# edamametechnologies/flodbadd

Hardware: AMD Instinct MI355X
Metric: Mpackets/s device-resident header parse + 5-tuple classify, 64B & IMIX frames (higher is better)
Workload: dtype u8; 1 GPU; C2: 1,048,576 x 64-B IPv4/TCP frames per GPU, device-resident (BASELINE configs[1]); rotated_batches=32, batches_per_launch_max=32, filter=GlobalOnly, parallelism=packet-index shards x1

## Files before the change

### flodbadd_amd/csrc/fb_capi.hip

```cpp
#include <stdarg.h>
#include <stdio.h>
#include <stdlib.h>
#include <string.h>

#include <algorithm>
#include <chrono>
#include <cmath>
#include <memory>
#include <mutex>
#include <new>
#include <thread>
#include <vector>

#include "fb_host.h"
#include "fb_internal.h"
#include "service_ports_default.inc"

using namespace fbk;

namespace fbk {

static thread_local char g_err[512] = "";

int set_err(int code, const char* fmt, ...) {
// ... 486 lines not shown
        return nullptr;
    }
    hipDeviceProp_t prop;
    if (hipGetDeviceProperties(&prop, device) != hipSuccess || strncmp(prop.gcnArchName, "gfx950", 6) != 0) {
        set_err(FB_ERR_NODEV, "device %d is not gfx950 (%s)", device, prop.gcnArchName);
        return nullptr;
    }
    DeviceGuard g(device);
    fb_ctx* c = new (std::nothrow) fb_ctx();
    if (!c) { set_err(FB_ERR_NOMEM, "fb_ctx"); return nullptr; }
    c->device = device;
    {
        int sb = 0;
        if (occupancy_parse_seg(&sb) != hipSuccess || sb < 1) sb = 1;
        c->seg_grid = std::min<uint32_t>((uint32_t)(sb * prop.multiProcessorCount), 1023u);
#ifndef FB_ASYNC_BPC
#define FB_ASYNC_BPC 1
#endif
        c->seg_grid_async = std::min<uint32_t>((uint32_t)(FB_ASYNC_BPC * prop.multiProcessorCount), c->seg_grid);
        int db = 0;
        if (occupancy_parse_dense(&db) != hipSuccess || db < 1) db = 1;
        c->dense_grid = std::min<uint32_t>((uint32_t)(db * prop.multiProcessorCount), 1023u);
    }
    c->h_cfg.reset(new (std::nothrow) DevConfig());
    bool ok = c->h_cfg != nullptr;
    if (ok) {
        memset(c->h_cfg.get(), 0, sizeof(DevConfig));
        memcpy(c->h_cfg->service_bitmap, cfg->service_bitmap ? cfg->service_bitmap : kDefaultServiceBitmap,
               FB_SERVICE_BITMAP_BYTES);
        c->h_cfg->filter = cfg->filter;
        set_lan(c->h_cfg.get(), cfg->lan_v6, cfg->n_lan_v6);
        c->h_cfg->n_own = cfg->n_own_ips;
        for (uint32_t i = 0; i < cfg->n_own_ips; ++i) c->h_cfg->own[i] = cfg->own_ips[i];
    }
    ok = ok && c->d_cfg.alloc(1) == hipSuccess;
    ok = ok && c->d_error.alloc(4) == hipSuccess && hipMemset(c->d_error, 0, 16) == hipSuccess;
    ok = ok && c->d_tick.alloc(kTickWords) == hipSuccess && hipMemset(c->d_tick, 0, kTickWords * 8ull) == hipSuccess;
    ok = ok && c->d_n.alloc(2) == hipSuccess;
    if (ok && cfg->flow_capacity > kFlowMaxCapacity) {
        set_err(FB_ERR_INVAL, "flow_capacity %llu > %llu slots", (unsigned long long)cfg->flow_capacity,
                (unsigned long long)kFlowMaxCapacity);
        ok = false;
    }
    if (ok && cfg->flow_capacity) {
        uint64_t cap = kFlowSlots;
        while (cap < cfg->flow_capacity) cap <<= 1;
        ok = table_alloc(c->tb, cap, nullptr) == nullptr &&
             hipMemset(c->tb.slots, 0, cap * sizeof(FlowSlot)) == hipSuccess &&
             c->mbox.alloc(1, hipHostMallocMapped) == hipSuccess;
        if (ok) memset(c->mbox.get(), 0, sizeof(FlowMailbox));
        c->grow = (cfg->flags & FB_CFG_FIXED_TABLE) == 0u;
        c->timed = (cfg->flags & FB_CFG_TIMED) != 0u;
        if (ok && c->timed)
            ok = plane_ensure(c, kPlaneTime, nullptr) == FB_OK;
        ok = ok && ensure_flow_scratch(c, cfg->max_batch_packets, nullptr) == FB_OK;
    }
    ok = ok && upload_cfg(c, nullptr) == FB_OK;
    if (!ok) {
        if (g_err[0] == 0) set_err(FB_ERR_NOMEM, "device allocation failed");
        fb_destroy(c);
        return nullptr;
    }
    return c;
}

int fb_destroy(fb_ctx* c) {
    if (!c) return set_err(FB_ERR_INVAL, "ctx is NULL");
    DeviceGuard g(c->device);
    (void)hipDeviceSynchronize();
    dnstrack_free(c->dns);
    histstore_free(c->hs);
    delete c;
    return FB_OK;
}

int fb_set_filter(fb_ctx* c, uint32_t filter) {
    if (!c || filter > FB_FILTER_ALL) return set_err(FB_ERR_INVAL, "bad ctx or filter");
    if (c->h_cfg->filter != filter) { c->h_cfg->filter = filter; c->cfg_dirty = true; }
    return FB_OK;
}

int fb_set_service_bitmap(fb_ctx* c, const uint8_t* bm) {
    if (!c || !bm) return set_err(FB_ERR_INVAL, "bad ctx or bitmap");
    memcpy(c->h_cfg->service_bitmap, bm, FB_SERVICE_BITMAP_BYTES);
    c->cfg_dirty = true;
    return FB_OK;
}

int fb_set_lan_v6(fb_ctx* c, const fb_lan_v6* nets, uint32_t n) {
    if (!c || n > FB_MAX_LAN_V6 || (n && !nets)) return set_err(FB_ERR_INVAL, "bad lan_v6 table");
    set_lan(c->h_cfg.get(), nets, n);
    c->cfg_dirty = true;
    return FB_OK;
}

int fb_set_stage_event(fb_ctx* c, void* event) {
    if (!c) return set_err(FB_ERR_INVAL, "ctx is NULL");
    c->stage_event = (hipEvent_t)event;
    return FB_OK;
}

int fb_set_frame_times(fb_ctx* c, const uint64_t* d_ts) {
    if (!c) return set_err(FB_ERR_INVAL, "ctx is NULL");
    if (!c->timed) return set_err(FB_ERR_INVAL, "the context was created without FB_CFG_TIMED");
    c->next_ts = reinterpret_cast<const unsigned long long*>(d_ts);
    return FB_OK;
}

static int timed_ready(fb_ctx* c) {
    if (c->timed && !c->next_ts)
        return set_err(FB_ERR_INVAL, "a timed context needs fb_set_frame_times before each update call");
    return FB_OK;
}

int fb_debug_set(fb_ctx* c, uint32_t knob, uint64_t value) {
    if (!c) return set_err(FB_ERR_INVAL, "ctx is NULL");
    switch (knob) {
        case FB_DEBUG_DENSE_STEAL_POLLS:
            c->steal_polls = (uint32_t)std::min<uint64_t>(value, 0xFFFFFFFFull);
            return FB_OK;
        case FB_DEBUG_DENSE_OFFSET_SKEW:
            if (value > 0xFFFFFFFFull) return set_err(FB_ERR_INVAL, "skew %llu >= 2^32", (unsigned long long)value);
            c->dn_skew = value;
            if (value) fprintf(stderr, "flodbadd_gpu: FB_DEBUG_DENSE_OFFSET_SKEW %llu active on this context (fault injection)\n",
                               (unsigned long long)value);
            return FB_OK;
        case FB_DEBUG_VIEW_DIRECT:
            c->view_direct = value != 0;
            return FB_OK;
        case FB_DEBUG_ZEEK_DIRECT:
            c->zeek_direct = value != 0;
            return FB_OK;
        default:
            return set_err(FB_ERR_INVAL, "unknown debug knob %u", knob);
    }
}

int fb_set_session_records(fb_ctx* c, int emit) {
    if (!c) return set_err(FB_ERR_INVAL, "ctx is NULL");
    c->emit_records = emit != 0;
    return FB_OK;
}

int fb_set_own_ips(fb_ctx* c, const fb_ip* ips, uint32_t n) {
    if (!c || n > FB_MAX_OWN_IPS || (n && !ips)) return set_err(FB_ERR_INVAL, "bad own-ip table");
    c->h_cfg->n_own = n;
    for (uint32_t i = 0; i < n; ++i) c->h_cfg->own[i] = ips[i];
    c->cfg_dirty = true;
    return FB_OK;
}

#ifdef FB_SEG_TRACE
static unsigned long long* g_strace = nullptr;
extern "C" __attribute__((visibility("default"))) int fb_seg_trace_last(unsigned long long* out) {
    if (!g_strace || hipDeviceSynchronize() != hipSuccess) return -1;
    return hipMemcpy(out, g_strace, 8u * 4u * 2048u, hipMemcpyDeviceToHost) == hipSuccess ? 0 : -1;
}
#endif
static int launch_seg(fb_ctx* c, const SegBatches& sb, uint32_t n_max, const fb_parsed_pkt* parsed, hipStream_t s,
                      bool want_parts = false, SegPass pass = SegPass::kSegments, fb_pkt_out* dense_out = nullptr,
                      fb_dns_out* dense_dns = nullptr) {
    int rc = reset_launch_scratch(c, s);
    if (!rc && want_parts && !c->part_target) rc = join_updates(c, s);
    if (!rc) rc = upload_cfg(c, s);
    if (!rc) rc = ensure_flow_scratch(c, n_max, s);
    if (rc) return rc;
    c->last_n = n_max;
    ParseParams p;
    memset(&p, 0, sizeof(p));
    p.pre = c->sc.cpre;
    p.dense_out = dense_out;
    p.dense_dns = dense_dns;
    p.parsed = parsed;
    p.n = parsed ? sb.b[0].n : 0u;
    p.rec_part = (want_parts && sb.count == 1u && c->tb.slots) ? (c->part_target ? c->part_target : c->rs.rec_part.get())
                                                              : nullptr;
    p.rec_ent = p.rec_part ? (c->ent_target ? c->ent_target : c->rs.rec_ent.get()) : nullptr;
    p.no_records = p.rec_part && !c->emit_records ? 1u : 0u;
    p.part_shift = c->tb.shift;
    c->part_recs = p.rec_part ? sb.b[0].out : nullptr;
    c->part_buf = p.rec_part;
    c->ent_buf = p.rec_ent;
    p.cfg = c->d_cfg;
    p.tick = c->d_tick;
    if (pass != SegPass::kDenseOut) {
        rc = guard_next_error_word(c, s);
        if (rc) return rc;
    }
    const uint32_t launch = pass == SegPass::kDenseOut ? c->epoch : ++c->epoch;
    p.error = c->d_error + (launch & 3u);
    p.error_next = c->d_error + ((launch + 1u) & 3u);
    const uint32_t waves = parse_seg_block_threads() / 64u;
    const uint32_t grid = std::max<uint32_t>(1u, std::min<uint32_t>(c->seg_grid, (sb.total_segs + waves - 1) / waves));
#ifdef FB_SEG_TRACE
    if (!g_strace && hipMalloc(&g_strace, 8u * 4u * 2048u) != hipSuccess) return set_err(FB_ERR_NOMEM, "trace");
    HIP_TRY(hipMemsetAsync(g_strace, 0, 8u * 4u * 2048u, s));
    p.dtrace = g_strace;
#endif
    HIP_TRY(launch_parse_seg(p, sb, grid, s, pass));
    return FB_OK;
}

static SegBatches one_batch(const uint8_t* frames, uint64_t frames_bytes, const uint32_t* offsets, uint32_t n,
                            fb_pkt_out* out, uint32_t* seg, uint8_t* cls, fb_batch_stats* stats) {
    SegBatches sb;
    memset(&sb, 0, sizeof(sb));
    sb.count = 1;
    SegBatch& B = sb.b[0];
    B.frames = frames;
    B.offsets = offsets;
    B.out = out;
    B.seg = seg;
    B.cls = cls;
    B.stats = stats;
    B.n = n;
    B.frames_bytes = (uint32_t)frames_bytes;
    sb.total_segs = (n + FB_SEG_FRAMES - 1) / FB_SEG_FRAMES;
    return sb;
}

int fb_parse_classify_seg_batches_dev(fb_ctx* c, const fb_seg_batch* batches, uint32_t count, void* stream) {
    if (!c || !batches || count == 0 || count > FB_MAX_SEG_BATCHES)
        return set_err(FB_ERR_INVAL, "ctx, batches and 1 <= count <= FB_MAX_SEG_BATCHES are required");
    SegBatches sb;
    memset(&sb, 0, sizeof(sb));
    uint64_t segs = 0;
    uint32_t n_max = 0;
    for (uint32_t k = 0; k < count; ++k) {
        const fb_seg_batch& x = batches[k];
        if (!x.d_stats) return set_err(FB_ERR_INVAL, "batch %u: d_stats is required", k);
        if (x.n > FB_MAX_BATCH_PACKETS) return set_err(FB_ERR_INVAL, "batch %u: n > FB_MAX_BATCH_PACKETS", k);
        if (x.frames_bytes > 0xFFFFFFFFull) return set_err(FB_ERR_INVAL, "batch %u: frames_bytes must be < 4 GiB", k);
        if (!x.d_offsets || (x.n && (!x.d_out || !x.d_seg)))
            return set_err(FB_ERR_INVAL, "batch %u: d_offsets, d_out and d_seg are required", k);
        if (x.n && x.frames_bytes && !x.d_frames) return set_err(FB_ERR_INVAL, "batch %u: d_frames is NULL", k);
        SegBatch& B = sb.b[k];
        B.frames = x.d_frames;
        B.offsets = x.d_offsets;
        B.out = x.d_out;
        B.seg = x.d_seg;
        B.cls = x.d_class;
        B.stats = x.d_stats;
        B.n = x.n;
        B.frames_bytes = (uint32_t)x.frames_bytes;
        B.seg_start = (uint32_t)segs;
        segs += (x.n + FB_SEG_FRAMES - 1) / FB_SEG_FRAMES;
        n_max = std::max(n_max, x.n);
    }
    if (segs > 0xFFFFFFFFull / FB_SEG_FRAMES) return set_err(FB_ERR_INVAL, "too many frames in one launch");
    sb.count = count;
    sb.total_segs = (uint32_t)segs;
    DeviceGuard g(c->device);
    return launch_seg(c, sb, n_max, nullptr, (hipStream_t)stream);
}

#ifdef FB_DN_TRACE
static unsigned long long* g_dtrace = nullptr;
extern "C" __attribute__((visibility("default"))) int fb_dense_trace_last(unsigned long long* out) {
    if (!g_dtrace || hipDeviceSynchronize() != hipSuccess) return -1;
    return hipMemcpy(out, g_dtrace, 8u * 4u * (8192u + 1024u), hipMemcpyDeviceToHost) == hipSuccess ? 0 : -1;
}
#endif
#ifdef FB_QUEUE_TRACE
static unsigned long long g_qtrace[kQTraceAll];
#endif
struct fb_seg_queue {
    int device = 0;
    uint32_t depth = 0;
    uint32_t slots = 0;
    PinnedBuf<QueueHost> h;
    DevBuf<QueueDev> d_ring;
    DevBuf<DevConfig> d_cfg;
    DevBuf<unsigned long long> d_tick;
    DevBuf<uint32_t> d_blk;
    DevBuf<uint32_t> d_head;
    DevBuf<uint32_t> d_err;
    DevBuf<unsigned long long> d_trace;
    DevStream stream;
    uint64_t submitted = 0;
    uint64_t limit = FB_QUEUE_MAX_SUBMISSIONS;
    bool launched = false;
    hipError_t gone = hipSuccess;
    uint32_t grid = 0;
    uint64_t idle_ns = 0;
    std::chrono::steady_clock::time_point created;
    bool not_resident = false;
    bool counted = false;
};
static std::mutex g_queue_mu;
static uint32_t g_queue_live[64];

static void queue_free(fb_seg_queue* q) {
    if (q->counted) {
        std::lock_guard<std::mutex> lk(g_queue_mu);
        --g_queue_live[q->device];
    }
    delete q;
}

static uint64_t hload(const unsigned long long* p) { return __atomic_load_n(p, __ATOMIC_ACQUIRE); }

static int queue_kernel_gone(fb_seg_queue* q, uint64_t spin, uint64_t every) {
    if (hload(&q->h->status) & kQueueExpired) return FB_OK;
    if (spin % every != every - 1u) return 1;
    const hipError_t e = hipStreamQuery(q->stream);
    if (e == hipErrorNotReady) {
        if (hload(&q->h->pad[3]) != q->grid &&
            (uint64_t)std::chrono::duration_cast<std::chrono::nanoseconds>(std::chrono::steady_clock::now() -
                                                                          q->created).count() > q->idle_ns) {
            q->not_resident = true;
            return FB_OK;
        }
        return 1;
    }
    q->gone = e;
    return FB_OK;
}

static int queue_gone_error(fb_seg_queue* q) {
    const QueueHost* h = q->h;
    if (q->not_resident)
        return set_err(FB_ERR_INTERNAL,
                       "the queue kernel's blocks are not all running (%llu of %u started within idle_ms): the "
                       "device's CUs are held by other work; destroy the queue",
                       (unsigned long long)hload(&h->pad[3]), q->grid);
    return set_err(FB_ERR_INTERNAL,
                   "the queue kernel has stopped (status %llu, stream: %s; a block left after %llu ticks idle "
                   "waiting for batch %llu (block %llu), tail %llu): destroy the queue",
                   (unsigned long long)hload(&h->status), hipGetErrorString(q->gone), (unsigned long long)hload(&h->pad[0]),
                   (unsigned long long)(hload(&h->pad[1]) & 0xFFFFFFFFu), (unsigned long long)(hload(&h->pad[1]) >> 32),
                   (unsigned long long)hload(&h->pad[2]));
}

fb_seg_queue* fb_seg_queue_create(fb_ctx* c, uint32_t depth, uint32_t idle_ms) {
    return fb_seg_queue_create_ex(c, depth, idle_ms, 0u);
}

fb_seg_queue* fb_seg_queue_create_ex(fb_ctx* c, uint32_t depth, uint32_t idle_ms, uint32_t flags) {
    if (flags & ~FB_QUEUE_SHARED) {
        set_err(FB_ERR_INVAL, "unknown queue flags 0x%x", flags);
        return nullptr;
    }
    if (!c) {
        set_err(FB_ERR_INVAL, "ctx is NULL");
        return nullptr;
    }
    if (depth == 0u) depth = 8u;
    if (depth > kQueueMax) {
        set_err(FB_ERR_INVAL, "depth %u > FB_QUEUE_MAX_DEPTH", depth);
// ... 1740 lines not shown
```

### flodbadd_amd/csrc/fb_parse.hip

```cpp
#include "fb_internal.h"

namespace fbk {

typedef uint32_t u32x4 __attribute__((ext_vector_type(4)));
typedef uint32_t u32x2 __attribute__((ext_vector_type(2)));

#ifndef FB_LD_AUX
#define FB_LD_AUX 0
#endif
#ifndef FB_ST_AUX
#define FB_ST_AUX 2
#endif

__device__ __forceinline__ u32x4 ld16(__amdgpu_buffer_rsrc_t r, uint32_t off) {
    return __builtin_amdgcn_raw_buffer_load_b128(r, off, 0, FB_LD_AUX);
}

__device__ __forceinline__ uint32_t be16_lo(uint32_t w) { return ((w & 0xffu) << 8) | ((w >> 8) & 0xffu); }
__device__ __forceinline__ uint32_t be16_hi(uint32_t w) { return ((w >> 8) & 0xff00u) | (w >> 24); }
__device__ __forceinline__ uint32_t bswap(uint32_t w) { return __builtin_bswap32(w); }

__device__ __forceinline__ uint32_t svc(const uint32_t* bm, uint32_t p) { return (bm[p >> 5] >> (p & 31)) & 1u; }

__device__ __forceinline__ uint32_t hist_char(uint32_t fl, uint32_t plen, bool orig) {
    uint32_t c;
    if ((fl & 0x02u) && !(fl & 0x10u)) c = 'S';
    else if ((fl & 0x02u) && (fl & 0x10u)) c = 'H';
    else if (fl & 0x01u) c = 'F';
    else if (fl & 0x04u) c = 'R';
    else if (plen > 0u) c = '>';
    else if (fl & 0x10u) c = 'A';
    else return '-';
    if (c == '>') return orig ? '>' : '<';
    return orig ? c : c + 32u;
}

#ifndef FB_HDR_ALIGNED
#define FB_HDR_ALIGNED 1
#endif
struct Hdr {
#if FB_HDR_ALIGNED
    u32x4 A, B, C;
    uint32_t E;
    uint32_t D0, D1;
#else
    u32x4 A, B, C;
    uint32_t Dz;
#endif
};

__device__ __forceinline__ void hdr_view(const Hdr& h, uint32_t o, u32x4& A, u32x4& B, u32x4& C, uint32_t& Dz) {
#if FB_HDR_ALIGNED
    const uint32_t s = (o + 10u) & 3u;
    auto al = [s](uint32_t hi, uint32_t lo) { return __builtin_amdgcn_alignbyte(hi, lo, s); };
    A = u32x4{al(h.A.y, h.A.x), al(h.A.z, h.A.y), al(h.A.w, h.A.z), al(h.B.x, h.A.w)};
    B = u32x4{al(h.B.y, h.B.x), al(h.B.z, h.B.y), al(h.B.w, h.B.z), al(h.C.x, h.B.w)};
    C = u32x4{al(h.C.y, h.C.x), al(h.C.z, h.C.y), al(h.C.w, h.C.z), al(h.E, h.C.w)};
    Dz = al(h.D1, h.D0);
#else
    (void)o;
    A = h.A;
    B = h.B;
    C = h.C;
    Dz = h.Dz;
#endif
}

struct Pkt {
    uint32_t cls;
    uint32_t w[14];
    bool tcp, v4, bad;
};

__device__ __forceinline__ void classify_session(const DevConfig* cfg, const DevConfig* gcfg, uint32_t proto,
                                                 uint32_t fam, const uint32_t (&src)[4], const uint32_t (&dst)[4],
                                                 uint32_t sport, uint32_t dport, uint32_t hasf, uint32_t flags,
                                                 uint32_t plen, uint32_t iplen, uint32_t idx, Pkt& k) {
    const uint32_t* bm = cfg->service_bitmap;
    k.tcp = proto == 6u;
    k.v4 = fam == 2u;
    const uint32_t S = svc(bm, sport), Dsv = svc(bm, dport);
    bool swap;
    if (S && !Dsv) {
        swap = true;
    } else if (S && Dsv) {
        const bool tf = hasf && proto == 6u && (flags & 0x02u);
        if (tf && !(flags & 0x10u)) swap = false;
        else if (tf && (flags & 0x10u)) swap = true;
        else swap = sport < dport;
    } else {
        swap = false;
    }
    const bool orig = !swap || (src[0] == dst[0] && src[1] == dst[1] && src[2] == dst[2] &&
                                src[3] == dst[3] && sport == dport);
    uint32_t ks[4], kd[4];
#pragma unroll
    for (int j = 0; j < 4; ++j) {
        ks[j] = swap ? dst[j] : src[j];
        kd[j] = swap ? src[j] : dst[j];
    }
    const uint32_t kport_s = swap ? dport : sport, kport_d = swap ? sport : dport;
    const bool lan_s = fam == 2u ? lan_v4(ks[0]) : lan_v6(cfg, gcfg, ks);
    const bool lan_d = fam == 2u ? lan_v4(kd[0]) : lan_v6(cfg, gcfg, kd);
    uint32_t meta = hasf;
    meta |= swap ? FB_META_SWAP : 0u;
    meta |= orig ? FB_META_ORIGINATOR : 0u;
    meta |= lan_s ? FB_META_LOCAL_SRC : 0u;
    meta |= lan_d ? FB_META_LOCAL_DST : 0u;
    meta |= own_ip(cfg, gcfg, fam, ks) ? FB_META_SELF_SRC : 0u;
    meta |= own_ip(cfg, gcfg, fam, kd) ? FB_META_SELF_DST : 0u;
    meta |= (swap ? S : Dsv) ? FB_META_DST_SERVICE : 0u;
    const uint32_t hc = hasf ? hist_char(flags, plen, orig) : 0u;
#pragma unroll
    for (int j = 0; j < 4; ++j) {
        k.w[j] = ks[j];
        k.w[4 + j] = kd[j];
    }
    k.w[8] = kport_s | (kport_d << 16);
    k.w[9] = proto | (fam << 8);
    k.w[10] = plen;
    k.w[11] = iplen;
    k.w[12] = flags | (meta << 8) | (hc << 16);
    k.w[13] = idx;
    const bool local = lan_s && lan_d;
    const uint32_t f = cfg->filter;
    const bool drop = (f == FB_FILTER_LOCAL_ONLY && !local) || (f == FB_FILTER_GLOBAL_ONLY && local);
    k.cls = drop ? FB_CLASS_FILTERED : FB_CLASS_SESSION;
}

__device__ __forceinline__ void process_frame(__amdgpu_buffer_rsrc_t r, const DevConfig* cfg,
                                              const DevConfig* gcfg, const Hdr& h, uint32_t o0, uint32_t o1,
                                              uint32_t fbytes, uint32_t idx, Pkt& k) {
    k.cls = FB_CLASS_DROP;
    k.tcp = false;
    k.v4 = false;
    const bool okoff = o1 >= o0 && o1 <= fbytes;
    k.bad = !okoff;
    const uint32_t L = okoff ? o1 - o0 : 0u;
    u32x4 A, B, C;
    uint32_t Dz;
    hdr_view(h, o0, A, B, C, Dz);
    if (L < 14u) return;
    const uint32_t et = be16_hi(A.x);
    const uint32_t n = L - 14u;
    uint32_t src[4] = {0u, 0u, 0u, 0u}, dst[4] = {0u, 0u, 0u, 0u};
    uint32_t l4off, l4len, proto, d0, d3, iplen, fam;
    if (et == 0x0800u) {
        if (n < 20u) return;
        const uint32_t ihl4 = (A.y & 0xfu) * 4u;
        const uint32_t tot = be16_hi(A.y);
        proto = (A.w >> 8) & 0xffu;
        const uint32_t start = ihl4 > 20u ? ihl4 : 20u;
        const uint32_t plen = tot > ihl4 ? tot - ihl4 : 0u;
        l4len = n > start ? min(start + plen, n) - start : 0u;
        l4off = 14u + start;
        src[0] = bswap(B.x);
        dst[0] = bswap(B.y);
        iplen = tot;
        fam = 2u;
        if (start == 20u) {
            d0 = B.z;
            d3 = C.y;
        } else {
            const u32x4 E = ld16(r, o0 + l4off);
            d0 = E.x;
            d3 = E.w;
        }
    } else if (et == 0x86DDu) {
        if (n < 40u) return;
        const uint32_t plen6 = be16_lo(A.z);
        proto = (A.z >> 16) & 0xffu;
        src[0] = bswap(A.w); src[1] = bswap(B.x); src[2] = bswap(B.y); src[3] = bswap(B.z);
        dst[0] = bswap(B.w); dst[1] = bswap(C.x); dst[2] = bswap(C.y); dst[3] = bswap(C.z);
        l4off = 54u;
        l4len = n > 40u ? min(40u + plen6, n) - 40u : 0u;
        iplen = plen6 + 40u;
        fam = 10u;
        d0 = C.w;
        d3 = Dz;
    } else {
        return;
    }
    uint32_t sport, dport, flags = 0u, hasf = 0u, plen;
    if (proto == 6u) {
        if (l4len < 20u) return;
        sport = be16_lo(d0);
        dport = be16_hi(d0);
        const uint32_t doff = (d3 & 0xffu) >> 4;
        flags = (d3 >> 8) & 0xffu;
        hasf = 1u;
        const uint32_t hs = doff > 5u ? doff * 4u : 20u;
        plen = l4len <= hs ? 0u : l4len - hs;
        if (sport == 53u || dport == 53u) {
            if (plen < 2u) return;
            k.cls = FB_CLASS_DNS;
            k.w[0] = idx;
            k.w[1] = o0 + l4off + hs + 2u;
            k.w[2] = plen - 2u;
            k.w[3] = 6u | (fam << 8);
            return;
        }
    } else if (proto == 17u) {
        if (l4len < 8u) return;
        sport = be16_lo(d0);
        dport = be16_hi(d0);
        plen = l4len - 8u;
        if (sport == 53u || dport == 53u) {
            k.cls = FB_CLASS_DNS;
            k.w[0] = idx;
            k.w[1] = o0 + l4off + 8u;
            k.w[2] = plen;
            k.w[3] = 17u | (fam << 8);
            return;
        }
    } else {
        return;
    }

    classify_session(cfg, gcfg, proto, fam, src, dst, sport, dport, hasf, flags, plen, iplen, idx, k);
}

constexpr uint32_t kFlagsProduct = 0u;
constexpr uint32_t kPartOut = 8u;
constexpr uint32_t kCountOnly = 16u;
constexpr uint32_t kDense = 32u;


__device__ __forceinline__ void load_headers1(__amdgpu_buffer_rsrc_t rs, uint32_t o, Hdr& h) {
#if FB_HDR_ALIGNED
    const uint32_t a = (o + 10u) & ~3u;
    h.A = ld16(rs, a);
    h.B = ld16(rs, a + 16u);
    h.C = ld16(rs, a + 32u);
    h.E = __builtin_amdgcn_raw_buffer_load_b32(rs, a + 48u, 0, FB_LD_AUX);
    const u32x2 d = __builtin_amdgcn_raw_buffer_load_b64(rs, a + 56u, 0, FB_LD_AUX);
    h.D0 = d.x;
    h.D1 = d.y;
#else
    h.A = ld16(rs, o + 10u);
    h.B = ld16(rs, o + 26u);
    h.C = ld16(rs, o + 42u);
    h.Dz = __builtin_amdgcn_raw_buffer_load_b32(rs, o + 66u, 0, FB_LD_AUX);
#endif
}

__device__ __forceinline__ void lds_barrier() { asm volatile("s_waitcnt lgkmcnt(0)\n\ts_barrier" ::: "memory"); }

#ifndef FB_SEG_WAVES
#define FB_SEG_WAVES 8
#endif
#ifndef FB_SEG_BPC
#define FB_SEG_BPC 3
#endif
#ifndef FB_SEG_DEPTH
#define FB_SEG_DEPTH 1
#endif
constexpr int kSegWaves = FB_SEG_WAVES;
constexpr int kSegDepth = FB_SEG_DEPTH;
constexpr int kSegThreads = 64 * kSegWaves;
constexpr uint32_t kSegBytes = 64u * 56u;

#ifdef FB_SEG_TRACE
constexpr uint32_t kSegTrBlocks = 2048u;
__device__ __forceinline__ unsigned long long seg_now() {
    unsigned long long t;
    asm volatile("s_memrealtime %0\n\ts_waitcnt lgkmcnt(0)" : "=s"(t)::"memory");
    return t;
}
#define SEGTR(stmt) do { stmt; } while (0)
#else
#define SEGTR(stmt) do { } while (0)
#endif
template <bool PARSED, uint32_t FLAGS = kFlagsProduct, bool MULTI = false>
__global__ __launch_bounds__(kSegThreads, kSegWaves * FB_SEG_BPC / 4) void k_parse_seg(const ParseParams P,
                                                                                      const SegBatches SB) {
    const uint32_t tid = threadIdx.x, lane = tid & 63u;
    const uint32_t wave = __builtin_amdgcn_readfirstlane(tid >> 6);
    const uint32_t G = gridDim.x, b = blockIdx.x;
    const uint32_t nseg = SB.total_segs;
    const uint32_t nb = MULTI ? SB.count : 1u;
    constexpr uint32_t kAcc = kMaxSegBatches * 10u;
    __shared__ uint4 s_cfg4[sizeof(DevConfig) / 16];
    constexpr uint32_t kStageU64 = (FLAGS & kPartOut) ? 64u * 8u : 64u * 7u;
    __shared__ __attribute__((aligned(16))) unsigned long long s_stage[kSegWaves][kStageU64];
    __shared__ uint32_t s_acc[kAcc + 1];
    const DevConfig* cfg = reinterpret_cast<const DevConfig*>(s_cfg4);
    const unsigned long long lmask = (1ull << lane) - 1ull;
    unsigned long long* stage = s_stage[wave];
    uint32_t a_s = 0u, a_d = 0u, a_f = 0u, a_t = 0u, a_4 = 0u, a_b = 0u, a_n = 0u;
    uint32_t a_k = 0u;
    if (tid <= kAcc) s_acc[tid] = 0u;
    SEGTR(if (tid == 0u && b < kSegTrBlocks) P.dtrace[4u * b] = seg_now());

    uint32_t k_q = 0u, k_h = 0u, k_s = 0u;
    auto batch_of = [&](uint32_t& k, uint32_t g) {
        if constexpr (MULTI)
            while (k + 1u < nb && g >= SB.b[k + 1u].seg_start) ++k;
        return k;
    };
    auto frames_rsrc = [&](uint32_t k) {
        return __builtin_amdgcn_make_buffer_rsrc((void*)SB.b[k].frames, (short)0, (int)SB.b[k].frames_bytes, 0x00020000);
    };

    typedef uint32_t u32x2 __attribute__((ext_vector_type(2)));
    constexpr uint32_t kOob = 0x80000000u;
    const uint32_t stride = G * kSegWaves;
    const __amdgpu_buffer_rsrc_t r_drop = __builtin_amdgcn_make_buffer_rsrc(SB.b[0].seg, (short)0, 0, 0x00020000);
    auto vmov = [](uint32_t x) {
        uint32_t y;
        asm volatile("v_mov_b32 %0, %1" : "=v"(y) : "v"(x));
        return y;
    };
    constexpr int D = kSegDepth;
    static_assert(D == 1, "one segment of header loads in flight (dynamic hand-out)");
    __shared__ uint32_t s_next;
    auto seg_of = [&](uint32_t L) { return b * kSegWaves + L % kSegWaves + (L / kSegWaves) * stride; };
    auto grab = [&]() {
        uint32_t v = 0u;
        if (lane == 0u) v = __hip_atomic_fetch_add(&s_next, 1u, __ATOMIC_RELAXED, __HIP_MEMORY_SCOPE_WORKGROUP);
        return __builtin_amdgcn_readfirstlane(v);
    };
    struct Set {
        Hdr h;
        uint2 c, q;
        unsigned long long p;
    };
    Set SS[D];
    uint4 pin[4];
    auto load_q = [&](uint32_t g, uint2& q) {
        const uint32_t k = batch_of(k_q, g);
        const uint32_t i = (g - SB.b[k].seg_start) * 64u + lane, n = SB.b[k].n;
        const uint32_t* off = SB.b[k].offsets;
        q = make_uint2(off[min(i, n)], off[min(i + 1u, n)]);
    };
    auto load_pre = [&](uint32_t g) {
        return P.pre[min(g, nseg - 1u)];
    };
    unsigned long long ppre = 0ull;
    auto fetch = [&](Set& X, uint32_t g_h, uint32_t next_q) {
        if constexpr ((FLAGS & kDense) != 0u) X.p = load_pre(g_h);
        load_headers1(frames_rsrc(batch_of(k_h, g_h)), X.q.x, X.h);
        X.c = make_uint2(vmov(X.q.x), vmov(X.q.y));
        load_q(next_q, X.q);
    };
    constexpr int kStores = (FLAGS & kCountOnly) ? 2 : (FLAGS & kDense) ? 6 : ((FLAGS & kPartOut) ? 13 : 8);
    auto dropped_stores = [&]() {
#pragma unroll
        for (int j = 0; j < kStores; ++j) __builtin_amdgcn_raw_buffer_store_b32(0u, r_drop, kOob + 64u * j, 0, 0);
    };
    auto load_parsed = [&](uint32_t sg) {
        if constexpr ((FLAGS & kDense) != 0u) ppre = load_pre(sg);
        const uint32_t sc = min(sg, (P.n - 1u) >> 6);
        const uint32_t left = P.n - sc * 64u;
        const __amdgpu_buffer_rsrc_t rp = __builtin_amdgcn_make_buffer_rsrc(
            (void*)(P.parsed + (size_t)sc * 64u), (short)0, (int)(min(left, 64u) * 56u), 0x00020000);
        const uint32_t o = min(lane, left - 1u) * 56u;
        const u32x4 x0 = __builtin_amdgcn_raw_buffer_load_b128(rp, o, 0, 0);
        const u32x4 x1 = __builtin_amdgcn_raw_buffer_load_b128(rp, o + 16u, 0, 0);
        const u32x4 x2 = __builtin_amdgcn_raw_buffer_load_b128(rp, o + 32u, 0, 0);
        const u32x2 x3 = __builtin_amdgcn_raw_buffer_load_b64(rp, o + 48u, 0, 0);
        pin[0] = make_uint4(x0.x, x0.y, x0.z, x0.w);
        pin[1] = make_uint4(x1.x, x1.y, x1.z, x1.w);
        pin[2] = make_uint4(x2.x, x2.y, x2.z, x2.w);
        pin[3] = make_uint4(x3.x, x3.y, 0u, 0u);
    };
    uint32_t Lc = wave, Ln = wave + kSegWaves;
    uint32_t sg = seg_of(Lc);
    if (tid == 0u) s_next = 2u * kSegWaves;
    constexpr uint32_t kCfg16 = kCfgLdsBytes / 16, kCfgIt = (kCfg16 + kSegThreads - 1) / kSegThreads;
    uint4 cfgv[kCfgIt];
    {
        const uint4* src = reinterpret_cast<const uint4*>(P.cfg);
#pragma unroll
        for (uint32_t it = 0; it < kCfgIt; ++it) cfgv[it] = src[min(tid + it * kSegThreads, kCfg16 - 1u)];
    }
    if constexpr (!PARSED) {
        load_q(sg, SS[0].q);
    } else {
        load_parsed(sg);
    }
#pragma unroll
    for (uint32_t it = 0; it < kCfgIt; ++it)
        if (tid + it * kSegThreads < kCfg16) s_cfg4[tid + it * kSegThreads] = cfgv[it];
    {
        const uint4* src = reinterpret_cast<const uint4*>(P.cfg);
        constexpr uint32_t kLanOff = offsetof(DevConfig, lan_v6) / 16, kOwnOff = offsetof(DevConfig, own) / 16;
        const uint32_t nl = P.cfg->n_lan_v6 * (sizeof(LanV6) / 16), no = P.cfg->n_own * (sizeof(fb_ip) / 16);
        for (uint32_t k = tid; k < nl; k += kSegThreads) s_cfg4[kLanOff + k] = src[kLanOff + k];
        for (uint32_t k = tid; k < no; k += kSegThreads) s_cfg4[kOwnOff + k] = src[kOwnOff + k];
        if (b == 0u && tid == 0u && !(FLAGS & kDense)) *P.error_next = 0u;
    }
    if constexpr (!PARSED) fetch(SS[0], sg, seg_of(Ln));
    dropped_stores();
    lds_barrier();
    auto flush = [&]() {
        const uint32_t a_tot = a_s + a_f;
        const uint32_t mine[10] = {a_s, a_f, a_d, a_b, a_t, a_tot - a_t, a_4, a_tot - a_4, a_tot, a_n - a_tot - a_d};
        if (lane < 10u) {
            uint32_t v = 0u;
#pragma unroll
            for (int k = 0; k < 10; ++k) v = lane == (uint32_t)k ? mine[k] : v;
            __hip_atomic_fetch_add(&s_acc[a_k * 10u + lane], v, __ATOMIC_RELAXED, __HIP_MEMORY_SCOPE_WORKGROUP);
        }
        a_s = a_d = a_f = a_t = a_4 = a_b = a_n = 0u;
    };
    auto step = [&](uint32_t sg, Set& X, uint32_t g_next, uint32_t g_after) {
            const uint32_t k = batch_of(k_s, sg);
            if (MULTI && k != a_k) {
                flush();
                a_k = k;
            }
            const SegBatch& B = SB.b[k];
            const uint32_t ls = sg - B.seg_start;
            const uint32_t i = ls * 64u + lane;
            const bool valid = i < B.n;
            Pkt kk;
            if constexpr (!PARSED) {
                process_frame(frames_rsrc(k), cfg, cfg, X.h, valid ? X.c.x : 1u, valid ? X.c.y : 0u, B.frames_bytes, i,
                              kk);
            } else {
                const uint4 a = pin[0], bb = pin[1], cc = pin[2], d = pin[3];
                const uint32_t src[4] = {a.x, a.y, a.z, a.w}, dst[4] = {bb.x, bb.y, bb.z, bb.w};
                const uint32_t proto = cc.y & 0xffu, fam = (cc.y >> 8) & 0xffu;
                kk.bad = false;
                kk.cls = FB_CLASS_DROP;
                kk.tcp = kk.v4 = false;
                const uint32_t hasf = (d.x & 0xff00u) != 0u ? 1u : 0u;
                if ((proto == 6u || proto == 17u) && (fam == 2u || fam == 10u))
                    classify_session(cfg, cfg, proto, fam, src, dst, cc.x & 0xffffu, cc.x >> 16, hasf,
                                     hasf ? d.x & 0xffu : 0u, cc.z, cc.w, d.y, kk);
            }
            const bool is_s = valid && kk.cls == FB_CLASS_SESSION;
            const bool is_d = valid && kk.cls == FB_CLASS_DNS;
            const bool is_f = valid && kk.cls == FB_CLASS_FILTERED;
            const bool counted = is_s || is_f;
            const unsigned long long m_sess = __ballot(is_s), m_dns = __ballot(is_d);
            const uint32_t cs = (uint32_t)__popcll(m_sess), cd = (uint32_t)__popcll(m_dns);
            if (is_s && !(FLAGS & kCountOnly)) {
                unsigned long long* dd = stage + (size_t)__popcll(m_sess & lmask) * 7;
    #pragma unroll
                for (int w = 0; w < 7; ++w)
                    dd[w] = (unsigned long long)kk.w[2 * w] | ((unsigned long long)kk.w[2 * w + 1] << 32);
            }
            __builtin_amdgcn_wave_barrier();
            unsigned long long pw = 0ull;
            if constexpr ((FLAGS & kDense) != 0u) pw = PARSED ? ppre : X.p;
            if constexpr (!PARSED) fetch(X, g_next, g_after);
            else load_parsed(g_next);
            if constexpr ((FLAGS & kCountOnly) != 0u) {
                const __amdgpu_buffer_rsrc_t r_seg =
                    __builtin_amdgcn_make_buffer_rsrc(B.seg, (short)0, (int)(((B.n + 63u) / 64u) * 4u), 0x00020000);
                const __amdgpu_buffer_rsrc_t r_cls =
                    __builtin_amdgcn_make_buffer_rsrc(B.cls, (short)0, B.cls ? (int)B.n : 0, 0x00020000);
                __builtin_amdgcn_raw_buffer_store_b32(cs | (cd << 16), r_seg, lane == 0u ? ls * 4u : kOob, 0, 0);
                __builtin_amdgcn_raw_buffer_store_b8((uint8_t)kk.cls, r_cls, valid ? i : kOob, 0, 0);
            } else if constexpr ((FLAGS & kDense) != 0u) {
                const uint32_t bs = (uint32_t)pw, bd = (uint32_t)(pw >> 32);
                const uint32_t words = cs * 7u, head = cs ? (bs & 1u) : 0u, body = (words - head) >> 1;
                const __amdgpu_buffer_rsrc_t r_out = __builtin_amdgcn_make_buffer_rsrc(
                    reinterpret_cast<uint8_t*>(P.dense_out) + (size_t)bs * 56u, (short)0, P.dense_out ? (int)(words * 8u) : 0,
                    0x00020000);
                const __amdgpu_buffer_rsrc_t r_dns = __builtin_amdgcn_make_buffer_rsrc(
                    P.dense_dns + bd, (short)0, P.dense_dns ? (int)(cd * 16u) : 0, 0x00020000);
        #pragma unroll
                for (int j = 0; j < 4; ++j) {
                    const uint32_t cc = lane + 64u * j;
                    const uint32_t src = head + 2u * min(cc, 223u - head);
                    const unsigned long long x = stage[src], y = stage[src + 1u];
                    const u32x4 v = {(uint32_t)x, (uint32_t)(x >> 32), (uint32_t)y, (uint32_t)(y >> 32)};
                    __builtin_amdgcn_raw_buffer_store_b128(v, r_out, cc < body ? head * 8u + cc * 16u : kOob, 0, FB_ST_AUX);
                }
                {
                    const bool h1 = head && lane == 0u, t1 = ((words - head) & 1u) && lane == 1u;
                    const uint32_t w = lane == 0u ? 0u : (words ? words - 1u : 0u);
                    const unsigned long long x = stage[w];
                    const u32x2 v = {(uint32_t)x, (uint32_t)(x >> 32)};
                    __builtin_amdgcn_raw_buffer_store_b64(v, r_out, (h1 || t1) ? w * 8u : kOob, 0, FB_ST_AUX);
                }
                {
                    const u32x4 v = {kk.w[0], kk.w[1], kk.w[2], kk.w[3]};
                    __builtin_amdgcn_raw_buffer_store_b128(v, r_dns, is_d ? 16u * (uint32_t)__popcll(m_dns & lmask) : kOob,
                                                           0, 0);
                }
            } else {
                const __amdgpu_buffer_rsrc_t r_out = __builtin_amdgcn_make_buffer_rsrc(
                    reinterpret_cast<uint8_t*>(B.out) + (size_t)ls * kSegBytes, (short)0, (int)kSegBytes, 0x00020000);
                const __amdgpu_buffer_rsrc_t r_rec = __builtin_amdgcn_make_buffer_rsrc(
                    reinterpret_cast<uint8_t*>(B.out) + (size_t)ls * kSegBytes, (short)0,
                    ((FLAGS & kPartOut) != 0u && P.no_records) ? 0 : (int)kSegBytes, 0x00020000);
                const __amdgpu_buffer_rsrc_t r_seg =
                    __builtin_amdgcn_make_buffer_rsrc(B.seg, (short)0, (int)(((B.n + 63u) / 64u) * 4u), 0x00020000);
                const __amdgpu_buffer_rsrc_t r_cls =
                    __builtin_amdgcn_make_buffer_rsrc(B.cls, (short)0, B.cls ? (int)B.n : 0, 0x00020000);
                const uint32_t words = cs * 7u, body = words >> 1;
        #pragma unroll
                for (int j = 0; j < 4; ++j) {
                    const uint32_t cc = lane + 64u * j;
                    const uint32_t src = min(cc, 223u);
                    const unsigned long long x = stage[2u * src], y = stage[2u * src + 1u];
                    const u32x4 v = {(uint32_t)x, (uint32_t)(x >> 32), (uint32_t)y, (uint32_t)(y >> 32)};
                    __builtin_amdgcn_raw_buffer_store_b128(v, r_rec, cc < body ? cc * 16u : kOob, 0, FB_ST_AUX);
                }
                {
                    const bool tail = (words & 1u) && lane == 0u;
                    const unsigned long long x = stage[words ? words - 1u : 0u];
                    const u32x2 v = {(uint32_t)x, (uint32_t)(x >> 32)};
                    __builtin_amdgcn_raw_buffer_store_b64(v, r_rec, tail ? (words - 1u) * 8u : kOob, 0, FB_ST_AUX);
                }
                {
                    const u32x4 v = {kk.w[0], kk.w[1], kk.w[2], kk.w[3]};
                    __builtin_amdgcn_raw_buffer_store_b128(
                        v, r_out, is_d ? kSegBytes - 16u * (1u + (uint32_t)__popcll(m_dns & lmask)) : kOob, 0, 0);
                }
                __builtin_amdgcn_raw_buffer_store_b32(cs | (cd << 16), r_seg, lane == 0u ? ls * 4u : kOob, 0, 0);
                __builtin_amdgcn_raw_buffer_store_b8((uint8_t)kk.cls, r_cls, valid ? i : kOob, 0, 0);
                if constexpr ((FLAGS & kPartOut) != 0u) {
                    const __amdgpu_buffer_rsrc_t r_part = __builtin_amdgcn_make_buffer_rsrc(
                        P.rec_part + (size_t)ls * 64u, (short)0, 256, 0x00020000);
                    const uint32_t key[10] = {kk.w[0], kk.w[1], kk.w[2], kk.w[3], kk.w[4],
                                              kk.w[5], kk.w[6], kk.w[7], kk.w[8], kk.w[9] & 0xFFFFu};
                    const uint32_t rank = (uint32_t)__popcll(m_sess & lmask);
                    const bool v6 = upd_ent_v6(kk.w[9]);
                    const unsigned long long m_v6 = __ballot(is_s && v6);
                    const uint32_t units = cs + (uint32_t)__popcll(m_v6);
                    const uint32_t part = part_of(flow_hash_words(key), P.part_shift);
                    uint32_t sv = (is_s ? part : 0x10000u) << 6 | lane;
#pragma unroll
                    for (uint32_t k = 2; k <= 64u; k <<= 1) {
#pragma unroll
                        for (uint32_t j = k >> 1; j > 0; j >>= 1) {
                            const uint32_t o = (uint32_t)__shfl_xor((int)sv, (int)j, 64);
                            const bool up = (lane & k) == 0u, lower = (lane & j) == 0u;
                            sv = (lower == up) ? min(sv, o) : max(sv, o);
                        }
                    }
                    const uint32_t src = sv & 63u;
                    const uint32_t sz = lane < cs ? ((m_v6 >> src) & 1ull ? 2u : 1u) : 0u;
                    uint32_t pre = sz;
#pragma unroll
                    for (int o = 1; o < 64; o <<= 1) {
                        const uint32_t y = (uint32_t)__shfl_up((int)pre, o, 64);
                        if (lane >= (uint32_t)o) pre += y;
                    }
                    const uint32_t uoff = (uint32_t)__builtin_amdgcn_ds_permute((int)(src * 4u), (int)(pre - sz));
                    const uint32_t pw = part | uoff << kRecUnitShift | (v6 ? kRecV6 : 0u);
                    __builtin_amdgcn_raw_buffer_store_b32(pw, r_part, is_s ? rank * 4u : kOob, 0, 0);
                    if (is_s) {
                        const uint32_t meta = (kk.w[12] >> 8) & 0xFFu;
                        const uint32_t hinfo = ((kk.w[12] >> 16) & 0xFFu) | ((kk.w[12] & 0xFFu) << 8) |
                                               ((meta & FB_META_HAS_FLAGS) ? 1u << 16 : 0u) | ((meta >> 3) & 0x1Fu) << 20;
                        const uint32_t aw = kk.w[9] | ((meta & FB_META_ORIGINATOR) ? 1u << 16 : 0u);
                        u32x4* e = reinterpret_cast<u32x4*>(stage + (size_t)uoff * 4u);
                        e[0] = u32x4{kk.w[0], kk.w[4], kk.w[8], aw};
                        e[1] = u32x4{kk.w[10], kk.w[11], kk.w[13], hinfo | rank << 26};
                        if (v6) {
                            e[2] = u32x4{kk.w[1], kk.w[2], kk.w[3], kk.w[5]};
                            e[3] = u32x4{kk.w[6], kk.w[7], 0u, 0u};
                        }
                    }
                    __builtin_amdgcn_wave_barrier();
                    const __amdgpu_buffer_rsrc_t r_ent = __builtin_amdgcn_make_buffer_rsrc(
                        P.rec_ent + (size_t)ls * 64u * kUpdEntU4, (short)0, (int)(units * 32u), 0x00020000);
#pragma unroll
                    for (uint32_t k = 0; k < kUpdEntU4; ++k) {
                        const uint32_t q = k * 64u + lane;
                        const u32x4 v = *reinterpret_cast<const u32x4*>(stage + (size_t)min(q, 255u) * 2u);
                        __builtin_amdgcn_raw_buffer_store_b128(v, r_ent, q * 16u, 0, 0);
                    }
                }
            }
            __builtin_amdgcn_wave_barrier();
            a_s += cs;
            a_d += cd;
            a_f += __popcll(__ballot(is_f));
            a_t += __popcll(__ballot(counted && kk.tcp));
            a_4 += __popcll(__ballot(counted && kk.v4));
            a_b += __popcll(__ballot(valid && kk.bad));
            a_n += __popcll(__ballot(valid));
    };
#ifdef FB_SEG_TRACE
    uint32_t steps_ = 0u;
#endif
    while (sg < nseg) {
        const uint32_t La = grab();
        const uint32_t g_next = seg_of(Ln);
        step(sg, SS[0], g_next, seg_of(La));
        Lc = Ln;
        Ln = La;
        sg = g_next;
        SEGTR(++steps_);
    }
    SEGTR(if (lane == 0u && b < kSegTrBlocks) {
        atomicMax(P.dtrace + 4u * b + 1u, seg_now());
        atomicAdd(P.dtrace + 4u * b + 2u, (unsigned long long)steps_);
    });
    if constexpr ((FLAGS & kDense) != 0u) return;
    {
        flush();
        asm volatile("s_waitcnt lgkmcnt(0)" ::: "memory");
        uint32_t arrived = 0u;
        if (lane == 0u) arrived = __hip_atomic_fetch_add(&s_acc[kAcc], 1u, __ATOMIC_RELAXED, __HIP_MEMORY_SCOPE_WORKGROUP);
        arrived = __shfl(arrived, 0, 64);
        if (arrived == (uint32_t)kSegWaves - 1u) {
            asm volatile("" ::: "memory");
            for (uint32_t t = lane; t < 5u * nb; t += 64u) {
                const uint32_t k = t / 5u, j = t - 5u * k;
                const unsigned long long lo = s_acc[k * 10u + 2u * j], hi = s_acc[k * 10u + 2u * j + 1u];
                unsigned long long* word = P.tick + k * 8u + j;
                const unsigned long long add = (1ull << 54) | (hi << 27) | lo;
                const unsigned long long old = __hip_atomic_fetch_add(word, add, __ATOMIC_RELAXED, __HIP_MEMORY_SCOPE_AGENT);
                if ((old >> 54) != (unsigned long long)G - 1u) continue;
                const unsigned long long tot = old + add, m27 = (1ull << 27) - 1ull;
                const unsigned long long f_lo = tot & m27, f_hi = (tot >> 27) & m27;
                __hip_atomic_store(word, 0ull, __ATOMIC_RELAXED, __HIP_MEMORY_SCOPE_AGENT);
                fb_batch_stats* S = SB.b[k].stats;
                if (!S) continue;
                if (j == 0u) {
                    S->n_session = f_lo;
                    S->n_filtered = f_hi;
                    S->new_sessions = 0ull;
                    S->updated_sessions = 0ull;
                    S->error = __hip_atomic_load(P.error, __ATOMIC_RELAXED, __HIP_MEMORY_SCOPE_AGENT);
                    S->reserved[0] = S->reserved[1] = S->reserved[2] = 0ull;
                } else if (j == 1u) {
                    S->n_dns = f_lo;
                    S->bad_offsets = f_hi;
                } else if (j == 2u) {
                    S->tcp_processed = f_lo;
                    S->udp_processed = f_hi;
                } else if (j == 3u) {
                    S->ipv4_processed = f_lo;
                    S->ipv6_processed = f_hi;
                } else {
                    S->total_processed = f_lo;
                    S->n_drop = f_hi;
                }
            }
        }
    }
    SEGTR(if (lane == 0u && b < kSegTrBlocks) atomicMax(P.dtrace + 4u * b + 3u, seg_now()));
}

#ifndef FB_DN_WAVES
#define FB_DN_WAVES 15
#endif
#ifndef FB_DN_TILE
#define FB_DN_TILE 16
#endif
#ifndef FB_DN_BPC
#define FB_DN_BPC 1
#endif
#ifndef FB_DN_LB
#define FB_DN_LB 1
#endif
#ifndef FB_DN_BUFS
#define FB_DN_BUFS 2
#endif
#ifndef FB_DN_SLEEP
#define FB_DN_SLEEP 1
#endif
constexpr int kDnWaves = FB_DN_WAVES;
constexpr uint32_t kDnTileSegs = FB_DN_TILE;
constexpr int kDnThreads = 64 * (kDnWaves + 1);
constexpr int kDnLb = FB_DN_LB;
constexpr uint32_t kDnBufs = FB_DN_BUFS;
constexpr uint32_t kDnSlotU64 = kSegBytes / 8u;
static_assert(kDnTileSegs <= 64u, "the store wave holds one segment count per lane");
constexpr unsigned long long kDnA = 1ull << 54, kDnP = 1ull << 55, kDn27 = (1ull << 27) - 1ull;
__device__ __forceinline__ unsigned long long dn_word(uint32_t ep, unsigned long long flag, unsigned long long pair) {
    return ((unsigned long long)ep << 56) | flag | (pair & kDn27) | (((pair >> 32) & kDn27) << 27);
}
__device__ __forceinline__ unsigned long long dn_pair(unsigned long long w) {
    return (w & kDn27) | (((w >> 27) & kDn27) << 32);
}
#ifdef FB_DN_TRACE
constexpr uint32_t kDnTrTiles = 8192u, kDnTrBlocks = 1024u;
__device__ __forceinline__ unsigned long long dn_now() {
    unsigned long long t;
    asm volatile("s_memrealtime %0\n\ts_waitcnt lgkmcnt(0)" : "=s"(t)::"memory");
    return t;
}
#define DNTR(stmt) do { stmt; } while (0)
#else
#define DNTR(stmt) do { } while (0)
#endif
struct DnLds {
    unsigned long long buf[kDnBufs][kDnTileSegs][kDnSlotU64];
    unsigned long long base[kDnBufs];
    uint32_t cnt[kDnBufs][kDnTileSegs];
    uint32_t pre[kDnBufs][kDnTileSegs];
    uint32_t done[kDnBufs];
    uint32_t copied[kDnBufs];
    uint32_t ready_round[kDnBufs];
    uint32_t free_round[kDnBufs];
    uint32_t next;
    uint32_t acc[11];
};

__global__ __launch_bounds__(kDnThreads, (FB_DN_BPC * kDnThreads + 255) / 256) void k_parse_dense(const ParseParams P,
                                                                                        const SegBatch B) {
    const uint32_t tid = threadIdx.x, lane = tid & 63u;
    const uint32_t wave = __builtin_amdgcn_readfirstlane(tid >> 6);
    const uint32_t G = gridDim.x, b = blockIdx.x;
    const uint32_t nt = P.ntiles, ep = P.dep, n = B.n;
    const uint32_t nseg = (n + 63u) / 64u;
    __shared__ uint4 s_cfg4[sizeof(DevConfig) / 16];
    __shared__ DnLds L;
    const DevConfig* cfg = reinterpret_cast<const DevConfig*>(s_cfg4);
    const unsigned long long lmask = (1ull << lane) - 1ull;
    constexpr uint32_t kOob = 0x80000000u;
    const __amdgpu_buffer_rsrc_t r_fr =
        __builtin_amdgcn_make_buffer_rsrc((void*)B.frames, (short)0, (int)B.frames_bytes, 0x00020000);
    const __amdgpu_buffer_rsrc_t r_cls = __builtin_amdgcn_make_buffer_rsrc(B.cls, (short)0, B.cls ? (int)n : 0, 0x00020000);
    const bool parser = wave < (uint32_t)kDnWaves;
    if (tid < kDnBufs) {
        L.done[tid] = 0u;
        L.copied[tid] = 0u;
        L.ready_round[tid] = ~0u;
        L.free_round[tid] = tid;
    }
    if (tid <= 10u) L.acc[tid] = 0u;
    if (tid == 0u) L.next = 2u * kDnWaves;
    DNTR(if (tid == 0u && b < kDnTrBlocks) P.dtrace[4u * kDnTrTiles + 4u * b] = dn_now());

    auto seg_of = [&](uint32_t Ls) { return (b + (Ls / kDnTileSegs) * G) * kDnTileSegs + Ls % kDnTileSegs; };
    auto grab = [&]() {
        uint32_t v = 0u;
        if (lane == 0u) v = __hip_atomic_fetch_add(&L.next, 1u, __ATOMIC_RELAXED, __HIP_MEMORY_SCOPE_WORKGROUP);
        return __builtin_amdgcn_readfirstlane(v);
    };
    auto load_q = [&](uint32_t g, uint2& q) {
        const uint32_t i = min(g, nseg) * 64u + lane;
        q = make_uint2(B.offsets[min(i, n)], B.offsets[min(i + 1u, n)]);
    };
    auto vmov = [](uint32_t x) {
        uint32_t y;
        asm volatile("v_mov_b32 %0, %1" : "=v"(y) : "v"(x));
        return y;
    };
    Hdr h;
    uint2 c = make_uint2(0u, 0u), q = make_uint2(0u, 0u);
    uint32_t Lc = wave, Ln = wave + kDnWaves;
    if (parser) load_q(seg_of(Lc), q);
    {
        constexpr uint32_t kCfg16 = kCfgLdsBytes / 16;
        const uint4* src = reinterpret_cast<const uint4*>(P.cfg);
        for (uint32_t k = tid; k < kCfg16; k += kDnThreads) s_cfg4[k] = src[k];
// ... 840 lines not shown
```

Measured before the change: 47600 Mpackets/s.

## Hoist IPv4-options L4 load early and cache per-batch descriptors in parse kernel

Issues the L4 header load for IPv4 frames with IP options speculatively at the top of process_frame, so its latency overlaps the rest of parsing instead of sitting as a dependent load later. Replaces the per-call linear batch_of search plus repeated SegBatch reads with cached per-stream descriptors that advance only at batch boundaries, cutting scalar loads in the hot loop. Also adds per-wave trace instrumentation that compiles only under FB_SEG_TRACE. For the 64B plain IPv4/TCP test frames the early-load path is never taken, and the wave-level ballot it adds is a small extra cost.

```diff
diff --git a/flodbadd_amd/csrc/fb_capi.hip b/flodbadd_amd/csrc/fb_capi.hip
--- a/flodbadd_amd/csrc/fb_capi.hip
+++ b/flodbadd_amd/csrc/fb_capi.hip
@@ -662,9 +662,14 @@
 
 #ifdef FB_SEG_TRACE
 static unsigned long long* g_strace = nullptr;
+constexpr size_t kSegTrBlockBytes = 8u * 4u * 2048u, kSegTrWaveBytes = 8u * 8u * 8192u;
 extern "C" __attribute__((visibility("default"))) int fb_seg_trace_last(unsigned long long* out) {
     if (!g_strace || hipDeviceSynchronize() != hipSuccess) return -1;
-    return hipMemcpy(out, g_strace, 8u * 4u * 2048u, hipMemcpyDeviceToHost) == hipSuccess ? 0 : -1;
+    return hipMemcpy(out, g_strace, kSegTrBlockBytes, hipMemcpyDeviceToHost) == hipSuccess ? 0 : -1;
+}
+extern "C" __attribute__((visibility("default"))) int fb_seg_trace_waves(unsigned long long* out) {
+    if (!g_strace || hipDeviceSynchronize() != hipSuccess) return -1;
+    return hipMemcpy(out, g_strace + kSegTrBlockBytes / 8u, kSegTrWaveBytes, hipMemcpyDeviceToHost) == hipSuccess ? 0 : -1;
 }
 #endif
 static int launch_seg(fb_ctx* c, const SegBatches& sb, uint32_t n_max, const fb_parsed_pkt* parsed, hipStream_t s,
@@ -703,8 +708,9 @@
     const uint32_t waves = parse_seg_block_threads() / 64u;
     const uint32_t grid = std::max<uint32_t>(1u, std::min<uint32_t>(c->seg_grid, (sb.total_segs + waves - 1) / waves));
 #ifdef FB_SEG_TRACE
-    if (!g_strace && hipMalloc(&g_strace, 8u * 4u * 2048u) != hipSuccess) return set_err(FB_ERR_NOMEM, "trace");
-    HIP_TRY(hipMemsetAsync(g_strace, 0, 8u * 4u * 2048u, s));
+    if (!g_strace && hipMalloc(&g_strace, kSegTrBlockBytes + kSegTrWaveBytes) != hipSuccess)
+        return set_err(FB_ERR_NOMEM, "trace");
+    HIP_TRY(hipMemsetAsync(g_strace, 0, kSegTrBlockBytes + kSegTrWaveBytes, s));
     p.dtrace = g_strace;
 #endif
     HIP_TRY(launch_parse_seg(p, sb, grid, s, pass));
diff --git a/flodbadd_amd/csrc/fb_parse.hip b/flodbadd_amd/csrc/fb_parse.hip
--- a/flodbadd_amd/csrc/fb_parse.hip
+++ b/flodbadd_amd/csrc/fb_parse.hip
@@ -128,6 +128,7 @@
     k.cls = drop ? FB_CLASS_FILTERED : FB_CLASS_SESSION;
 }
 
+template <bool OPT_EARLY = true>
 __device__ __forceinline__ void process_frame(__amdgpu_buffer_rsrc_t r, const DevConfig* cfg,
                                               const DevConfig* gcfg, const Hdr& h, uint32_t o0, uint32_t o1,
                                               uint32_t fbytes, uint32_t idx, Pkt& k) {
@@ -140,6 +141,15 @@
     u32x4 A, B, C;
     uint32_t Dz;
     hdr_view(h, o0, A, B, C, Dz);
+    const bool opt = OPT_EARLY && L >= 34u && be16_hi(A.x) == 0x0800u && (A.y & 0xfu) > 5u;
+    uint32_t Eo0 = 0u, Eo3 = 0u;
+    if (OPT_EARLY && __ballot(opt) != 0ull) {
+        if (opt) {
+            const u32x4 E = ld16(r, o0 + 14u + (A.y & 0xfu) * 4u);
+            asm volatile("v_mov_b32 %0, %1" : "=v"(Eo0) : "v"(E.x));
+            asm volatile("v_mov_b32 %0, %1" : "=v"(Eo3) : "v"(E.w));
+        }
+    }
     if (L < 14u) return;
     const uint32_t et = be16_hi(A.x);
     const uint32_t n = L - 14u;
@@ -161,6 +171,9 @@
         if (start == 20u) {
             d0 = B.z;
             d3 = C.y;
+        } else if constexpr (OPT_EARLY) {
+            d0 = Eo0;
+            d3 = Eo3;
         } else {
             const u32x4 E = ld16(r, o0 + l4off);
             d0 = E.x;
@@ -261,7 +274,7 @@
 constexpr uint32_t kSegBytes = 64u * 56u;
 
 #ifdef FB_SEG_TRACE
-constexpr uint32_t kSegTrBlocks = 2048u;
+constexpr uint32_t kSegTrBlocks = 2048u, kSegTrWaves = 8192u;
 __device__ __forceinline__ unsigned long long seg_now() {
     unsigned long long t;
     asm volatile("s_memrealtime %0\n\ts_waitcnt lgkmcnt(0)" : "=s"(t)::"memory");
@@ -293,13 +306,43 @@
     SEGTR(if (tid == 0u && b < kSegTrBlocks) P.dtrace[4u * b] = seg_now());
 
     uint32_t k_q = 0u, k_h = 0u, k_s = 0u;
-    auto batch_of = [&](uint32_t& k, uint32_t g) {
-        if constexpr (MULTI)
-            while (k + 1u < nb && g >= SB.b[k + 1u].seg_start) ++k;
-        return k;
-    };
-    auto frames_rsrc = [&](uint32_t k) {
-        return __builtin_amdgcn_make_buffer_rsrc((void*)SB.b[k].frames, (short)0, (int)SB.b[k].frames_bytes, 0x00020000);
+    auto next_start = [&](uint32_t k) { return k + 1u < nb ? SB.b[k + 1u].seg_start : ~0u; };
+    auto advance = [&](uint32_t& k, uint32_t& x, uint32_t g) {
+        if constexpr (MULTI) {
+            if (g < x) return false;
+            do x = next_start(++k);
+            while (g >= x);
+            return true;
+        }
+        return false;
+    };
+    struct DescS {
+        const uint8_t* frames;
+        fb_pkt_out* out;
+        uint32_t* seg;
+        uint8_t* cls;
+        uint32_t n, frames_bytes, seg_start;
+    };
+    struct DescH {
+        const uint8_t* frames;
+        uint32_t frames_bytes;
+    };
+    struct DescQ {
+        const uint32_t* offsets;
+        uint32_t n, seg_start;
+    };
+    auto desc_s = [&](uint32_t k) {
+        const SegBatch& B = SB.b[k];
+        return DescS{B.frames, B.out, B.seg, B.cls, B.n, B.frames_bytes, B.seg_start};
+    };
+    auto desc_h = [&](uint32_t k) { return DescH{SB.b[k].frames, SB.b[k].frames_bytes}; };
+    auto desc_q = [&](uint32_t k) { return DescQ{SB.b[k].offsets, SB.b[k].n, SB.b[k].seg_start}; };
+    DescS d_s = desc_s(0u);
+    DescH d_h = desc_h(0u);
+    DescQ d_q = desc_q(0u);
+    uint32_t x_s = MULTI ? next_start(0u) : ~0u, x_h = x_s, x_q = x_s;
+    auto frames_rsrc = [&](const uint8_t* frames, uint32_t frames_bytes) {
+        return __builtin_amdgcn_make_buffer_rsrc((void*)frames, (short)0, (int)frames_bytes, 0x00020000);
     };
 
     typedef uint32_t u32x2 __attribute__((ext_vector_type(2)));
@@ -328,9 +371,9 @@
     Set SS[D];
     uint4 pin[4];
     auto load_q = [&](uint32_t g, uint2& q) {
-        const uint32_t k = batch_of(k_q, g);
-        const uint32_t i = (g - SB.b[k].seg_start) * 64u + lane, n = SB.b[k].n;
-        const uint32_t* off = SB.b[k].offsets;
+        if (advance(k_q, x_q, g)) d_q = desc_q(k_q);
+        const uint32_t i = (g - d_q.seg_start) * 64u + lane, n = d_q.n;
+        const uint32_t* off = d_q.offsets;
         q = make_uint2(off[min(i, n)], off[min(i + 1u, n)]);
     };
     auto load_pre = [&](uint32_t g) {
@@ -339,7 +382,8 @@
     unsigned long long ppre = 0ull;
     auto fetch = [&](Set& X, uint32_t g_h, uint32_t next_q) {
         if constexpr ((FLAGS & kDense) != 0u) X.p = load_pre(g_h);
-        load_headers1(frames_rsrc(batch_of(k_h, g_h)), X.q.x, X.h);
+        if (advance(k_h, x_h, g_h)) d_h = desc_h(k_h);
+        load_headers1(frames_rsrc(d_h.frames, d_h.frames_bytes), X.q.x, X.h);
         X.c = make_uint2(vmov(X.q.x), vmov(X.q.y));
         load_q(next_q, X.q);
     };
@@ -391,6 +435,10 @@
         if (b == 0u && tid == 0u && !(FLAGS & kDense)) *P.error_next = 0u;
     }
     if constexpr (!PARSED) fetch(SS[0], sg, seg_of(Ln));
+#ifdef FB_SEG_TRACE
+    uint32_t steps_ = 0u;
+    unsigned long long tr_wait = 0ull, tr_drain = 0ull, tr_work = 0ull, tr_trip = 0ull, tr_fetch = 0ull;
+#endif
     dropped_stores();
     lds_barrier();
     auto flush = [&]() {
@@ -405,19 +453,35 @@
         a_s = a_d = a_f = a_t = a_4 = a_b = a_n = 0u;
     };
     auto step = [&](uint32_t sg, Set& X, uint32_t g_next, uint32_t g_after) {
-            const uint32_t k = batch_of(k_s, sg);
-            if (MULTI && k != a_k) {
+#ifdef FB_SEG_TRACE
+            unsigned long long tr_here = 0ull;
+            if constexpr (!PARSED) {
+                const unsigned long long t0 = seg_now();
+                asm volatile("s_waitcnt vmcnt(%0)" ::"n"(2 + kStores) : "memory");
+                tr_here = seg_now();
+                tr_wait += tr_here - t0;
+                if (steps_) tr_trip += tr_here - tr_fetch;
+#ifdef FB_SEG_TRACE_DRAIN
+                asm volatile("s_waitcnt vmcnt(0)" ::: "memory");
+                const unsigned long long t1 = seg_now();
+                tr_drain += t1 - tr_here;
+                tr_here = t1;
+#endif
+            }
+#endif
+            if (advance(k_s, x_s, sg)) {
                 flush();
-                a_k = k;
-            }
-            const SegBatch& B = SB.b[k];
+                a_k = k_s;
+                d_s = desc_s(k_s);
+            }
+            const DescS& B = d_s;
             const uint32_t ls = sg - B.seg_start;
             const uint32_t i = ls * 64u + lane;
             const bool valid = i < B.n;
             Pkt kk;
             if constexpr (!PARSED) {
-                process_frame(frames_rsrc(k), cfg, cfg, X.h, valid ? X.c.x : 1u, valid ? X.c.y : 0u, B.frames_bytes, i,
-                              kk);
+                process_frame<(FLAGS & kPartOut) == 0u>(frames_rsrc(B.frames, B.frames_bytes), cfg, cfg, X.h,
+                                                        valid ? X.c.x : 1u, valid ? X.c.y : 0u, B.frames_bytes, i, kk);
             } else {
                 const uint4 a = pin[0], bb = pin[1], cc = pin[2], d = pin[3];
                 const uint32_t src[4] = {a.x, a.y, a.z, a.w}, dst[4] = {bb.x, bb.y, bb.z, bb.w};
@@ -446,6 +510,12 @@
             unsigned long long pw = 0ull;
             if constexpr ((FLAGS & kDense) != 0u) pw = PARSED ? ppre : X.p;
             if constexpr (!PARSED) fetch(X, g_next, g_after);
+#ifdef FB_SEG_TRACE
+            if constexpr (!PARSED) {
+                tr_fetch = seg_now();
+                tr_work += tr_fetch - tr_here;
+            }
+#endif
             else load_parsed(g_next);
             if constexpr ((FLAGS & kCountOnly) != 0u) {
                 const __amdgpu_buffer_rsrc_t r_seg =
@@ -579,7 +649,7 @@
             a_n += __popcll(__ballot(valid));
     };
 #ifdef FB_SEG_TRACE
-    uint32_t steps_ = 0u;
+    const unsigned long long tr_loop = seg_now();
 #endif
     while (sg < nseg) {
         const uint32_t La = grab();
@@ -593,6 +663,16 @@
     SEGTR(if (lane == 0u && b < kSegTrBlocks) {
         atomicMax(P.dtrace + 4u * b + 1u, seg_now());
         atomicAdd(P.dtrace + 4u * b + 2u, (unsigned long long)steps_);
+        const uint32_t w = b * kSegWaves + wave;
+        if (w < kSegTrWaves) {
+            unsigned long long* tw = P.dtrace + 4u * kSegTrBlocks + 8u * w;
+            tw[0] = tr_wait;
+            tw[1] = tr_drain;
+            tw[2] = tr_work;
+            tw[3] = tr_trip;
+            tw[4] = seg_now() - tr_loop;
+            tw[5] = steps_;
+        }
     });
     if constexpr ((FLAGS & kDense) != 0u) return;
     {
```

Measured after the change: 48320 Mpackets/s (median of 6 runs). 1.5% higher.
